# jessicabonnie/dandd

Hardware: AMD Instinct MI355X
Metric: Gbp/s sketched over k-sweep (higher is better)
Workload: dtype u64; 1 GPU; cfg2: 10 x 50 Mbp synthetic FASTA on this GPU (10 over 1 GPU(s)) resident in HBM, HLL log2m=14, k-sweep 4-40 (K=37), leaf sketches + root union + all cardinalities + delta; genomes_per_gpu=10, bases_per_genome=50000000, kmin=4, kmax=40, log2m=14, parallelism=genomes sharded over 1 GPU(s)

## Files before the change

dandd_amd/build.py:

```python
import os
import subprocess
import sys

HERE = os.path.dirname(os.path.abspath(__file__))
CSRC = os.path.join(HERE, "csrc")
LIBDIR = os.path.join(HERE, "lib")
LIB = os.path.join(LIBDIR, "libdandd_hip.so")
SOURCES = ["dd_api.hip", "dd_k2_api.hip", "dd_exact_api.hip", "dd_ingest.hip", "dd_plan.hip", "dd_pack.hip", "dd_sweep.hip", "dd_union.hip", "dd_gram.hip", "dd_leaveout.hip", "dd_extend.hip", "dd_subsets.hip", "dd_pscan.hip", "dd_synth.hip", "dd_exact.hip", "dd_exact_sched.hip", "dd_ginflate.hip", "dd_fastq.hip"]
HEADERS = ["dd_common.h", "dd_ctx.h", "dd_io.h", "dd_inflate.h", "dd_kernels.h", "dd_plan.h", os.path.join("..", "..", "include", "dandd_hip.h")]
FLAGS = [
    "-O3",
    "--offload-arch=gfx950",
    "-std=c++17",
    "-fPIC",
    "-shared",
    "-ffp-contract=off",
    "-Wall",
    "-Wno-unused-function",
]


def hipcc():
    for cand in (os.environ.get("HIPCC"), "/opt/rocm/bin/hipcc", "hipcc"):
        if cand and (os.path.isabs(cand) and os.path.exists(cand) or not os.path.isabs(cand)):
            return cand
    raise RuntimeError("hipcc not found")


OBJDIR = os.path.join(HERE, "build", "obj")
COMPILE_FLAGS = [f for f in FLAGS if f != "-shared"]


def needs_build():
    if not os.path.exists(LIB):
        return True
    t = os.path.getmtime(LIB)
    deps = [os.path.join(CSRC, s) for s in SOURCES + HEADERS] + [os.path.abspath(__file__)]
    return any(os.path.getmtime(d) > t for d in deps)


BINDIR = os.path.join(HERE, "bin")
CLI = os.path.join(BINDIR, "dashing")
CLI_SRC = os.path.join(CSRC, "dd_cli.c")
FUSED_PARALLEL = os.path.join(BINDIR, "fused", "parallel")


def build_cli(force=False):
    inc = os.path.join(HERE, "..", "include")
    deps = [CLI_SRC, os.path.join(inc, "dandd_hip.h"), LIB]
    if (not force and os.path.exists(CLI) and os.path.exists(FUSED_PARALLEL)
            and all(os.path.getmtime(d) <= min(os.path.getmtime(CLI), os.path.getmtime(FUSED_PARALLEL)) for d in deps)):
        return CLI
    os.makedirs(os.path.dirname(FUSED_PARALLEL), exist_ok=True)
    cmd = [os.environ.get("CC", "gcc"), "-std=c99", "-O2", "-Wall", "-Wextra", "-pedantic", "-I" + inc, CLI_SRC, "-o", CLI + ".tmp",
           "-L" + LIBDIR, "-ldandd_hip", "-lz", "-Wl,-rpath,$ORIGIN/../lib", "-Wl,-rpath,$ORIGIN/../../lib", "-Wl,-rpath,/opt/rocm/lib",
           "-Wl,-rpath-link," + LIBDIR]
    subprocess.check_call(cmd)
    os.replace(CLI + ".tmp", CLI)
    import shutil
    shutil.copy2(CLI, FUSED_PARALLEL + ".tmp")
    os.replace(FUSED_PARALLEL + ".tmp", FUSED_PARALLEL)
    return CLI


def _stale(obj, src):
    if not os.path.exists(obj):
        return True
    t = os.path.getmtime(obj)
    return any(os.path.getmtime(d) > t for d in [src, os.path.abspath(__file__)] + [os.path.join(CSRC, h) for h in HEADERS])


def build(force=False, extra=(), verbose=False, jobs=None):
    if not force and not needs_build():
        return LIB
    os.makedirs(LIBDIR, exist_ok=True)
    os.makedirs(OBJDIR, exist_ok=True)
    cc = hipcc()
    todo, objs = [], []
    for s in SOURCES:
        src, obj = os.path.join(CSRC, s), os.path.join(OBJDIR, s.replace(".hip", ".o"))
        objs.append(obj)
        if force or extra or _stale(obj, src):
            todo.append([cc] + COMPILE_FLAGS + list(extra) + ["-c", src, "-o", obj])
    jobs = jobs or max(1, min(len(todo), (os.cpu_count() or 2) - 1, int(os.environ.get("DD_BUILD_JOBS", "6"))))
    running = []
    for cmd in todo:
        if verbose:
            print(" ".join(cmd), file=sys.stderr)
        running.append((cmd, subprocess.Popen(cmd, cwd=CSRC)))
        while len([1 for _, p in running if p.poll() is None]) >= jobs:
            running[0][1].wait()
            running = [r for r in running if r[1].poll() is None] + [r for r in running if r[1].poll() not in (None, 0)]
            if any(p.poll() not in (None, 0) for _, p in running):
                break
    bad = [cmd for cmd, p in running if p.wait() != 0]
    if bad:
        raise subprocess.CalledProcessError(1, bad[0])
    link = [cc, "--offload-arch=gfx950", "-shared", "-fPIC", "-o", LIB + ".tmp"] + objs + ["-lz", "-ldl", "-lpthread"]
    if verbose:
        print(" ".join(link), file=sys.stderr)
    subprocess.check_call(link, cwd=CSRC)
    os.replace(LIB + ".tmp", LIB)
    return LIB


if __name__ == "__main__":
    extra = []
    if "--save-temps" in sys.argv:
        os.makedirs(OBJDIR, exist_ok=True)
        extra += ["-save-temps=obj"]
    build(force="--force" in sys.argv, extra=extra, verbose=True)
    print(LIB)
    print(build_cli(force="--force" in sys.argv))
```

dandd_amd/csrc/dd_sweep.hip:

```cpp
#include "dd_common.h"
#include "dd_kernels.h"

#include <atomic>

namespace dd {
namespace {

extern __shared__ __attribute__((aligned(16))) uint8_t g_lds[];

DD_D uint32_t ffbh(uint32_t x) {
    uint32_t r;
    asm("v_ffbh_u32 %0, %1" : "=v"(r) : "v"(x));
    return r;
}
DD_D uint32_t mul_lo(uint32_t a, uint32_t c) {
    uint32_t r;
    asm("v_mul_lo_u32 %0, %1, %2" : "=v"(r) : "v"(a), "s"(c));
    return r;
}
template <int SH>
DD_D uint64_t lshl_add64(uint64_t a, uint64_t b) {
    uint64_t r;
    asm("v_lshl_add_u64 %0, %1, %2, %3" : "=v"(r) : "v"(a), "n"(SH), "v"(b));
    return r;
}
template <bool HI_ZERO>
DD_D uint64_t mul64_c32(uint64_t x, uint32_t C, uint64_t addend) {
    const uint32_t lo = (uint32_t)x, hi = (uint32_t)(x >> 32);
    const uint64_t pr = (uint64_t)lo * C + addend;
    if (HI_ZERO) return pr;
    const uint32_t ph = (uint32_t)(pr >> 32) + mul_lo(hi, C);
    return ((uint64_t)ph << 32) | (uint32_t)pr;
}

template <bool HI_ZERO>
DD_D uint64_t wang64_fast(uint64_t x) {
    x = mul64_c32<HI_ZERO>(x, 0x1FFFFFu, ~0ull);
    x ^= x >> 24;
    x = mul64_c32<false>(x, 265u, 0ull);
    x ^= x >> 14;
    x = lshl_add64<2>(lshl_add64<2>(x, x), x);
    x ^= x >> 28;
    return lshl_add64<0>(x << 31, x);
}

DD_D void lds_starts_at_zero() {
    if ((uint32_t)(uintptr_t)(__attribute__((address_space(3))) uint8_t*)g_lds != 0u) __builtin_trap();
}

struct RegsLds {
    uint32_t slot;
    using Addr = uint32_t;
    DD_D Addr at(uint32_t hi, int p) const { return __builtin_amdgcn_alignbit(slot, hi, 32 - p); }
    DD_D static uint32_t shift(Addr a) { return (a & 3u) * 8u; }
    DD_D uint32_t bound(Addr a) const { return *(const __attribute__((address_space(3))) uint8_t*)(uintptr_t)a; }
    DD_D static uint32_t load32(Addr a) { return *(const __attribute__((address_space(3))) uint32_t*)(uintptr_t)(a & ~3u); }
    DD_D static uint32_t cas32(Addr a, uint32_t expect, uint32_t desired) {
        return atomicCAS(reinterpret_cast<uint32_t*>(g_lds + (a & ~3u)), expect, desired);
    }
};
struct RegsGlobal {
    uint8_t* base;
    using Addr = uint8_t*;
    DD_D Addr at(uint32_t hi, int p) const { return base + (hi >> (32 - p)); }
    DD_D static uint32_t shift(Addr a) { return ((uint32_t)(uintptr_t)a & 3u) * 8u; }
    DD_D static uint8_t* word(Addr a) {
        return static_cast<uint8_t*>(__builtin_assume_aligned(a - ((uintptr_t)a & 3u), 4));
    }
    DD_D uint32_t bound(Addr a) const { return gload1_fresh(a); }
    DD_D static uint32_t load32(Addr a) { return gload4_fresh(word(a)); }
    DD_D static uint32_t cas32(Addr a, uint32_t expect, uint32_t desired) { return gcas32(word(a), expect, desired); }
};

DD_D uint4 load16_fresh(const uint8_t* p) {
    const uint8_t* q = static_cast<const uint8_t*>(__builtin_assume_aligned(p, 16));
    const unsigned long long a = gload8_fresh(q), b = gload8_fresh(q + 8);
    return make_uint4((uint32_t)a, (uint32_t)(a >> 32), (uint32_t)b, (uint32_t)(b >> 32));
}
DD_D uint32_t load4_fresh(const uint32_t* p) { return gload4_fresh(p); }

struct Probe {
    uint32_t hi, lz, hiw, lo;
};
DD_D Probe probe(uint64_t h, int p) {
    const uint32_t hi = (uint32_t)(h >> 32), lo = (uint32_t)h;
    Probe r;
    r.hi = hi;
    r.hiw = __builtin_amdgcn_alignbit(hi, lo, 32 - p);
    r.lz = ffbh(r.hiw);
    r.lo = lo;
    return r;
}
DD_D uint32_t rho_of(const Probe& q, int p) {
    uint32_t rho = q.lz + 1;
    if (__builtin_expect(__any(q.hiw == 0), 0)) {
        if (q.hiw == 0) rho = 33u + (uint32_t)__builtin_clz((q.lo << p) | (1u << (p - 1)));
    }
    return rho;
}
template <typename R>
DD_D uint32_t cas_raise(typename R::Addr a, uint32_t old, uint32_t rho) {
    const uint32_t sh = R::shift(a);
    while (true) {
        const uint32_t cur = (old >> sh) & 0xFFu;
        if (rho <= cur) return cur;
        const uint32_t prev = R::cas32(a, old, old + ((rho - cur) << sh));
        if (prev == old) return rho;
        old = prev;
    }
}
template <typename R>
DD_D void raise(const R&, typename R::Addr a, const Probe& q, int p) {
    (void)cas_raise<R>(a, R::load32(a), rho_of(q, p));
}

constexpr uint32_t kQueueEntries = 128;
DD_D uint32_t min4(uint32_t w) {
    const uint32_t a = w & 0xFFu, b = (w >> 8) & 0xFFu, c = (w >> 16) & 0xFFu, d = w >> 24;
    const uint32_t ab = a < b ? a : b, cd = c < d ? c : d;
    return ab < cd ? ab : cd;
}
template <typename R>
DD_D void hll_update(const R& regs, uint64_t h, int p) {
    const Probe q = probe(h, p);
    const typename R::Addr a = regs.at(q.hi, p);
    if (q.lz >= regs.bound(a)) raise(regs, a, q, p);
}
template <typename R>
DD_D void hll_update2(const R& r0, uint64_t h0, const R& r1, uint64_t h1, int p) {
    const Probe qa = probe(h0, p), qb = probe(h1, p);
    const typename R::Addr a = r0.at(qa.hi, p), b = r1.at(qb.hi, p);
    const uint32_t c0 = r0.bound(a), c1 = r1.bound(b);
    if ((qa.lz >= c0) | (qb.lz >= c1)) {
        if (qa.lz >= c0) raise(r0, a, qa, p);
        if (qb.lz >= c1) raise(r1, b, qb, p);
    }
}

DD_D uint32_t pairrev32(uint32_t x) {
    x = __builtin_bitreverse32(x);
    return ((x >> 1) & 0x55555555u) | ((x & 0x55555555u) << 1);
}
DD_D uint64_t pack64(uint32_t hi, uint32_t lo) { return ((uint64_t)hi << 32) | lo; }

template <int KC>
struct Windows;

template <>
struct Windows<0> {
    uint32_t fw = 0, rc = 0;
    DD_D void prime(const uint4& hc) {
        fw = pairrev32(hc.w);
        rc = ~hc.w;
    }
    DD_D void push(uint32_t c) {
        fw = (fw << 2) | c;
        rc = (rc >> 2) | ((3u - c) << 30);
    }
    template <bool CANON>
    DD_D uint64_t hash(int k) const {
        const uint32_t f = (k == 16) ? fw : (fw & ((1u << (2 * k)) - 1u));
        if (!CANON) return wang64_fast<true>(f);
        const uint32_t r = rc >> (32 - 2 * k);
        return wang64_fast<true>(f < r ? f : r);
    }
};

template <>
struct Windows<1> {
    uint64_t fw = 0, rc = 0;
    DD_D void prime(const uint4& hc) {
        fw = pack64(pairrev32(hc.z), pairrev32(hc.w));
        rc = ~pack64(hc.w, hc.z);
    }
    DD_D void push(uint32_t c) {
        fw = (fw << 2) | c;
        rc = (rc >> 2) | ((uint64_t)(3u - c) << 62);
    }
    template <bool CANON>
    DD_D uint64_t hash(int k) const {
        const uint32_t mhi = (k == 32) ? ~0u : ((1u << (2 * k - 32)) - 1u);
        const uint64_t f = pack64((uint32_t)(fw >> 32) & mhi, (uint32_t)fw);
        if (!CANON) return wang64_fast<false>(f);
        const uint64_t r = rc >> (64 - 2 * k);
        return wang64_fast<false>(f < r ? f : r);
    }
};

template <>
struct Windows<5> {
    uint32_t fl = 0, fh = 0, rl = 0, rh = 0;
    DD_D void prime(const uint4& hc) {
        fh = pairrev32(hc.z);
        fl = pairrev32(hc.w);
        rh = ~hc.w;
        rl = ~hc.z;
    }
    DD_D void push(uint32_t c) {
        fh = __builtin_amdgcn_alignbit(fh, fl, 30);
        fl = (fl << 2) | c;
        rl = __builtin_amdgcn_alignbit(rh, rl, 2);
        rh = (rh >> 2) | ((3u - c) << 30);
    }
    template <bool CANON>
    DD_D uint64_t hash(int k) const {
        const uint32_t mhi = (k == 32) ? ~0u : ((1u << (2 * k - 32)) - 1u);
        const uint64_t f = pack64(fh & mhi, fl);
        if (!CANON) return wang64_fast<false>(f);
        const uint64_t r = pack64(rh, rl) >> (64 - 2 * k);
        return wang64_fast<false>(f < r ? f : r);
    }
};

template <>
struct Windows<3> {
    uint64_t fl = 0, rt = 0;
    uint32_t fh = 0, rb = 0;
    DD_D void prime(const uint4& hc) {
        fl = pack64(pairrev32(hc.z), pairrev32(hc.w));
        fh = pairrev32(hc.y);
        rt = ~pack64(hc.w, hc.z);
        rb = ~hc.y;
    }
    DD_D void push(uint32_t c) {
        fh = __builtin_amdgcn_alignbit(fh, (uint32_t)(fl >> 32), 30);
        fl = (fl << 2) | c;
        rb = __builtin_amdgcn_alignbit((uint32_t)rt, rb, 2);
        rt = (rt >> 2) | ((uint64_t)(3u - c) << 62);
    }
    template <bool CANON>
    DD_D uint64_t hash(int k) const {
        const int hb = 2 * k - 64;
        const uint32_t ah = (hb == 32) ? fh : (fh & ((1u << hb) - 1u));
        uint32_t hi = ah;
        uint64_t lo = fl;
        if (CANON) {
            const uint32_t s = 96u - 2u * (uint32_t)k;
            const uint32_t r3 = (uint32_t)(rt >> 32), r2 = (uint32_t)rt;
            const uint32_t bh = r3 >> s;
            const uint64_t bl = ((uint64_t)__builtin_amdgcn_alignbit(r3, r2, s) << 32) |
                                __builtin_amdgcn_alignbit(r2, rb, s);
            const bool f_lt = (ah < bh) | ((ah == bh) & (fl < bl));
            hi = f_lt ? ah : bh;
            lo = f_lt ? fl : bl;
        }
        const uint64_t hg = (uint64_t)hi * 0x7F4A7C15u + ((uint64_t)(hi * 0x9E3779B9u) << 32);
        return wang64_fast<false>(lo ^ hg);
    }
};

template <>
struct Windows<6> {
    uint32_t f0 = 0, f1 = 0, f2 = 0;
    uint32_t r0 = 0, r1 = 0, r2 = 0;
    DD_D void prime(const uint4& hc) {
        f0 = pairrev32(hc.w);
        f1 = pairrev32(hc.z);
        f2 = pairrev32(hc.y);
        r2 = ~hc.w;
        r1 = ~hc.z;
        r0 = ~hc.y;
    }
    DD_D void push(uint32_t c) {
        f2 = __builtin_amdgcn_alignbit(f2, f1, 30);
        f1 = __builtin_amdgcn_alignbit(f1, f0, 30);
        f0 = (f0 << 2) | c;
        r0 = __builtin_amdgcn_alignbit(r1, r0, 2);
        r1 = __builtin_amdgcn_alignbit(r2, r1, 2);
        r2 = (r2 >> 2) | ((3u - c) << 30);
    }
    template <bool CANON>
    DD_D uint64_t hash(int k) const {
        const int hb = 2 * k - 64;
        const uint32_t ah = (hb == 32) ? f2 : (f2 & ((1u << hb) - 1u));
        const uint64_t fl = pack64(f1, f0);
        uint32_t hi = ah;
        uint64_t lo = fl;
        if (CANON) {
            const uint32_t s = 96u - 2u * (uint32_t)k;
            const uint32_t bh = r2 >> s;
            const uint64_t bl = pack64(__builtin_amdgcn_alignbit(r2, r1, s), __builtin_amdgcn_alignbit(r1, r0, s));
            const bool f_lt = (ah < bh) | ((ah == bh) & (fl < bl));
            hi = f_lt ? ah : bh;
            lo = f_lt ? fl : bl;
        }
        const uint64_t hg = (uint64_t)hi * 0x7F4A7C15u + ((uint64_t)(hi * 0x9E3779B9u) << 32);
        return wang64_fast<false>(lo ^ hg);
    }
};

template <>
struct Windows<7> {
    uint32_t f0 = 0, f1 = 0, f2 = 0, f3 = 0;
    uint32_t r0 = 0, r1 = 0, r2 = 0, r3 = 0;
    DD_D void prime(const uint4& hc) {
        f0 = pairrev32(hc.w);
        f1 = pairrev32(hc.z);
        f2 = pairrev32(hc.y);
        f3 = pairrev32(hc.x);
        r3 = ~hc.w;
        r2 = ~hc.z;
        r1 = ~hc.y;
        r0 = ~hc.x;
    }
    DD_D void push(uint32_t c) {
        f3 = __builtin_amdgcn_alignbit(f3, f2, 30);
        f2 = __builtin_amdgcn_alignbit(f2, f1, 30);
        f1 = __builtin_amdgcn_alignbit(f1, f0, 30);
        f0 = (f0 << 2) | c;
        r0 = __builtin_amdgcn_alignbit(r1, r0, 2);
        r1 = __builtin_amdgcn_alignbit(r2, r1, 2);
        r2 = __builtin_amdgcn_alignbit(r3, r2, 2);
        r3 = (r3 >> 2) | ((3u - c) << 30);
    }
    template <bool CANON>
    DD_D uint64_t hash(int k) const {
        const int hb = 2 * k - 96;
        const uint32_t mh = (hb == 32) ? ~0u : ((1u << hb) - 1u);
        const uint64_t ah = pack64(f3 & mh, f2);
        const uint64_t al = pack64(f1, f0);
        if (!CANON) return wang64_fast<false>(fold128(ah, al));
        const uint32_t s = 128u - 2u * (uint32_t)k;
        const uint64_t bh = pack64(r3 >> s, __builtin_amdgcn_alignbit(r3, r2, s));
        const uint64_t bl = pack64(__builtin_amdgcn_alignbit(r2, r1, s), __builtin_amdgcn_alignbit(r1, r0, s));
        const bool f_lt = (ah < bh) | ((ah == bh) & (al < bl));
        return wang64_fast<false>(fold128(f_lt ? ah : bh, f_lt ? al : bl));
    }
};

template <int KC, bool CANON, bool CHECK, typename Win, typename MakeRegs>
DD_D void sweep_token(const Win& win, int run, int kfirst, int nk, int p, const MakeRegs& slot) {
    int j = 0;
#pragma unroll 1
    for (; j + 1 < nk; j += 2) {
        const int k = kfirst + j;
        if (!CHECK || run >= k + 1)
            hll_update2(slot(j), win.template hash<CANON>(k), slot(j + 1), win.template hash<CANON>(k + 1), p);
        else if (run >= k)
            hll_update(slot(j), win.template hash<CANON>(k), p);
    }
    if (j < nk && (!CHECK || run >= kfirst + j)) hll_update(slot(j), win.template hash<CANON>(kfirst + j), p);
}

template <int KC, bool CANON>
__global__ __launch_bounds__(1024) void sweep_kernel(const SweepGenome* __restrict__ genomes,
                                                    const SweepJob* __restrict__ jobs, int p) {
    lds_starts_at_zero();
    const SweepJob job = jobs[blockIdx.x];
    const SweepGenome g = genomes[job.genome];
    const int nk = job.nk, kfirst = job.kfirst;
    const uint32_t m = 1u << p;
    const unsigned long long ntok = gload8u(g.ntok);
    uint8_t* const slab = g.regs + ((size_t)job.krow << p);

    struct TileIn {
        uint4 hc, sc;
        uint2 hb, sb;
        bool live;
    };
    auto fetch = [&](unsigned tile, TileIn& t) {
        const unsigned long long seg = (unsigned long long)tile * blockDim.x + threadIdx.x;
        t.live = tile < job.tile_end && seg * kSegTokens < ntok;
        t.hc = make_uint4(0, 0, 0, 0);
        t.hb = make_uint2(~0u, ~0u);
        t.sc = make_uint4(0, 0, 0, 0);
        t.sb = make_uint2(~0u, ~0u);
        if (!t.live) return;
        if (seg > 0) {
            t.hc = gload16(g.codes + (seg - 1) * 4);
            t.hb = gload8(g.bad + (seg - 1) * 2);
        }
        t.sc = gload16(g.codes + seg * 4);
        t.sb = gload8(g.bad + seg * 2);
    };
    TileIn next;
    fetch(job.tile_begin, next);

    {
        uint4* z = reinterpret_cast<uint4*>(g_lds);
        const uint32_t n16 = (uint32_t)nk * (m >> 4);
        for (uint32_t i = threadIdx.x; i < n16; i += blockDim.x) z[i] = load16_fresh(slab + (size_t)i * 16);
    }
    __syncthreads();

    const int kmaxg = kfirst + nk - 1;
    auto lds_slot = [](int j) { return RegsLds{(uint32_t)j}; };

    for (unsigned tile = job.tile_begin; tile < job.tile_end; ++tile) {
        const TileIn cur = next;
        fetch(tile + 1, next);
        if (!cur.live) continue;
        const uint4 hc = cur.hc, sc = cur.sc;
        const uint2 hb = cur.hb, sb = cur.sb;
        const uint32_t cw[4] = {sc.x, sc.y, sc.z, sc.w};
        Windows<KC == 2 ? 7 : KC> win;
        win.prime(hc);
        if (__all((hb.x | hb.y | sb.x | sb.y) == 0u)) {
#pragma unroll
            for (int w = 0; w < 4; ++w) {
#pragma unroll 1
                for (int i = 0; i < 16; ++i) {
                    win.push((cw[w] >> (2 * i)) & 3u);
                    sweep_token<KC, CANON, false>(win, 0, kfirst, nk, p, lds_slot);
                }
            }
            continue;
        }
        int run = hb.y ? __builtin_clz(hb.y) : 32 + (hb.x ? __builtin_clz(hb.x) : 32);
#pragma unroll
        for (int w = 0; w < 4; ++w) {
            const uint32_t bw = ((w & 2) ? sb.y : sb.x) >> ((w & 1) * 16);
#pragma unroll 1
            for (int i = 0; i < 16; ++i) {
                const uint32_t c = (cw[w] >> (2 * i)) & 3u;
                run = ((bw >> i) & 1u) ? 0 : run + 1;
                win.push(c);
                if (__all(run >= kmaxg)) sweep_token<KC, CANON, false>(win, run, kfirst, nk, p, lds_slot);
                else sweep_token<KC, CANON, true>(win, run, kfirst, nk, p, lds_slot);
            }
        }
    }
    __syncthreads();

    const uint4* l4 = reinterpret_cast<const uint4*>(g_lds);
    uint32_t* gw = reinterpret_cast<uint32_t*>(slab);
    const uint32_t n16 = (uint32_t)nk * (m >> 4);
    for (uint32_t i = threadIdx.x; i < n16; i += blockDim.x) {
        const uint4 lv = l4[i];
        const uint4 gv = load16_fresh(slab + (size_t)i * 16);
        const uint32_t l[4] = {lv.x, lv.y, lv.z, lv.w};
        const uint32_t o[4] = {gv.x, gv.y, gv.z, gv.w};
#pragma unroll
        for (int q = 0; q < 4; ++q) {
            uint32_t old = o[q];
            uint32_t mx = bmax4(old, l[q]);
            while (mx != old) {
                uint32_t prev = gcas32(&gw[4 * i + q], old, mx);
                if (prev == old) break;
                old = prev;
                mx = bmax4(old, l[q]);
            }
        }
    }
}

__constant__ int c_bitmap_off[kBitmapMaxK + 2] = {0, bitmap_offset(1), bitmap_offset(2), bitmap_offset(3),
                                                 bitmap_offset(4), bitmap_offset(5), bitmap_offset(6),
                                                 bitmap_offset(7), bitmap_offset(8), bitmap_offset(9),
                                                 kBitmapWords};
static_assert(kBitmapMaxK == 9 && bitmap_offset(9) + bitmap_words(9) == kBitmapWords &&
              kBitmapWords + kBitmapMaxK < kBitmapStride, "bitmap layout");

template <bool CANON>
__global__ __launch_bounds__(1024) __attribute__((amdgpu_num_sgpr(72))) void bitmap_kernel(const SweepGenome* __restrict__ genomes,
                                                     const SweepJob* __restrict__ jobs) {
    const SweepJob job = jobs[blockIdx.x];
    const SweepGenome g = genomes[job.genome];
    const int kfirst = job.kfirst, klast = job.kfirst + job.nk - 1;
    const unsigned long long ntok = gload8u(g.ntok);
    const int w0 = c_bitmap_off[kfirst], w1 = c_bitmap_off[klast + 1];
    uint32_t* const bits = reinterpret_cast<uint32_t*>(g_lds) - w0;
    uint32_t kmask = __builtin_amdgcn_readfirstlane(((2u << klast) - 1u) & ~((1u << kfirst) - 1u));
    uint32_t* const complete = g.bitmap + kBitmapWords;
    __shared__ uint32_t have[kBitmapMaxK + 2];
    __shared__ uint32_t flagged;
    if (threadIdx.x == 0) {
        uint32_t f = 0;
        for (int k = kfirst; k <= klast; ++k)
            if (load4_fresh(complete + k)) f |= 1u << k;
        flagged = f;
    }
    if (threadIdx.x <= kBitmapMaxK) have[threadIdx.x] = 0;
    __syncthreads();
    kmask = __builtin_amdgcn_readfirstlane(kmask & ~flagged);
    if (kmask == 0u) return;
    for (int i = w0 + (int)threadIdx.x; i < w1; i += blockDim.x) {
        const uint32_t v = load4_fresh(&g.bitmap[i]);
        bits[i] = v;
        if (v) {
            int k = kfirst;
            for (int j = kfirst + 1; j <= klast; ++j) k = (i >= c_bitmap_off[j]) ? j : k;
            atomicAdd(&have[k], (uint32_t)__builtin_popcount(v));
        }
    }
    __syncthreads();
    auto all_of = [](int k) { return CANON ? (1u << (2 * k - 1)) + ((k & 1) ? 0u : (1u << (k - 1))) : (1u << (2 * k)); };
    for (int k = kfirst; k <= klast; ++k) {
        if (have[k] == all_of(k)) {
            kmask &= ~(1u << k);
            if (threadIdx.x == 0) gstore4(complete + k, 1u);
        }
    }
    kmask = __builtin_amdgcn_readfirstlane(kmask);
    if (kmask == 0u) return;

    const int prime = klast - 1;
    for (unsigned tile = job.tile_begin; tile < job.tile_end; ++tile) {
        const unsigned long long seg = (unsigned long long)tile * blockDim.x + threadIdx.x;
        if (seg * kSegTokens >= ntok) continue;
        uint32_t fw = 0, rc = 0;
        int run = 0;
        if (seg > 0) {
            const uint4 hc = gload16(g.codes + (seg - 1) * 4);
            const uint2 hb = gload8(g.bad + (seg - 1) * 2);
            const uint32_t cw = hc.w, bw = hb.y >> 16;
#pragma unroll 1
            for (int i = 16 - prime; i < 16; ++i) {
                const uint32_t c = (cw >> (2 * i)) & 3u;
                run = ((bw >> i) & 1u) ? 0 : run + 1;
                fw = (fw << 2) | c;
                rc = (rc >> 2) | ((3u - c) << 30);
            }
        }
        const uint4 sc = gload16(g.codes + seg * 4);
        const uint2 sb = gload8(g.bad + seg * 2);
        const uint32_t cws[4] = {sc.x, sc.y, sc.z, sc.w};
#pragma unroll
        for (int w = 0; w < 4; ++w) {
            const uint32_t bw = ((w & 2) ? sb.y : sb.x) >> ((w & 1) * 16);
#pragma unroll 1
            for (int i = 0; i < 16; ++i) {
                const uint32_t c = (cws[w] >> (2 * i)) & 3u;
                run = ((bw >> i) & 1u) ? 0 : run + 1;
                fw = (fw << 2) | c;
                rc = (rc >> 2) | ((3u - c) << 30);
                uint32_t xs[kBitmapMaxK + 1], seen[kBitmapMaxK + 1];
                uint32_t all_seen = 1u;
#pragma unroll
                for (int k = 1; k <= kBitmapMaxK; ++k) {
                    if (!((kmask >> k) & 1u)) continue;
                    uint32_t x = fw & ((1u << (2 * k)) - 1u);
                    if (CANON) {
                        const uint32_t r = rc >> (32 - 2 * k);
                        x = x < r ? x : r;
                    }
                    xs[k] = x;
                    seen[k] = bits[bitmap_offset(k) + (x >> 5)];
                    all_seen &= seen[k] >> (x & 31u);
                }
                if (!(all_seen & 1u)) {
#pragma unroll
                    for (int k = 1; k <= kBitmapMaxK; ++k) {
                        if (!((kmask >> k) & 1u) || run < k) continue;
                        if (!((seen[k] >> (xs[k] & 31u)) & 1u))
                            atomicOr(&bits[bitmap_offset(k) + (xs[k] >> 5)], 1u << (xs[k] & 31u));
                    }
                }
            }
        }
    }
    __syncthreads();
    if (threadIdx.x <= kBitmapMaxK) have[threadIdx.x] = 0;
    __syncthreads();
    for (int i = w0 + (int)threadIdx.x; i < w1; i += blockDim.x) {
        const uint32_t mine = bits[i], theirs = load4_fresh(&g.bitmap[i]);
        if (mine & ~theirs) gor32(&g.bitmap[i], mine);
        int k = kfirst;
        for (int j = kfirst + 1; j <= klast; ++j) k = (i >= c_bitmap_off[j]) ? j : k;
        if (mine | theirs) atomicAdd(&have[k], (uint32_t)__builtin_popcount(mine | theirs));
    }
    __syncthreads();
    if (threadIdx.x >= (unsigned)kfirst && threadIdx.x <= (unsigned)klast && have[threadIdx.x] == all_of((int)threadIdx.x))
        gstore4(complete + threadIdx.x, 1u);
}

template <bool CANON_UNUSED>
__global__ __launch_bounds__(1024) void bitmap_finish_kernel(const SweepGenome* __restrict__ genomes,
                                                            int kfirst, int kmin, int p, int tile_log2) {
    lds_starts_at_zero();
    const SweepGenome g = genomes[blockIdx.y];
    const int k = kfirst + (int)blockIdx.x;
    const uint32_t tile = 1u << tile_log2, b = blockIdx.z;
    const uint32_t* bm = g.bitmap + c_bitmap_off[k];
    const int nw = c_bitmap_off[k + 1] - c_bitmap_off[k];
    if (gridDim.z > 1 && nw <= 512) {
        if (b != 0) return;
        uint8_t* const row = g.regs + ((size_t)(k - kmin) << p);
        for (int w = threadIdx.x; w < nw; w += blockDim.x) {
            uint32_t v = gload4(bm + w);
            while (v) {
                const uint32_t bit = (uint32_t)__builtin_ctz(v);
                v &= v - 1;
                hll_update(RegsGlobal{row}, wang64_fast<true>(((uint32_t)w << 5) | bit), p);
            }
        }
        return;
    }
    uint8_t* const out = g.regs + ((size_t)(k - kmin) << p) + (size_t)b * tile;
    uint4* z = reinterpret_cast<uint4*>(g_lds);
    for (uint32_t i = threadIdx.x; i < (tile >> 4); i += blockDim.x) z[i] = make_uint4(0, 0, 0, 0);
    __syncthreads();
    for (int w = threadIdx.x; w < nw; w += blockDim.x) {
        uint32_t v = gload4(bm + w);
        while (v) {
            const uint32_t bit = (uint32_t)__builtin_ctz(v);
            v &= v - 1;
            const Probe q = probe(wang64_fast<true>(((uint32_t)w << 5) | bit), p);
            const uint32_t idx = q.hi >> (32 - p);
            if ((idx >> tile_log2) != b) continue;
            const uint32_t a = idx & (tile - 1u), rho = rho_of(q, p);
            const uint32_t wd = RegsLds::load32(a);
            if (rho > ((wd >> RegsLds::shift(a)) & 0xFFu)) (void)cas_raise<RegsLds>(a, wd, rho);
        }
    }
    __syncthreads();
    const uint4* l4 = reinterpret_cast<const uint4*>(g_lds);
    for (uint32_t i = threadIdx.x; i < (tile >> 4); i += blockDim.x) gstore16(out + (size_t)i * 16, l4[i]);
}


template <bool CANON>
DD_D uint32_t bigmap_index(uint32_t fw, uint32_t rc, int k) {
    if (!CANON) return fw;
    if (k & 1) {
        const uint32_t y = ((fw >> k) & 1u) ? rc : fw;
        return ((y >> (k + 1)) << k) | (y & ((1u << k) - 1u));
    }
    return fw < rc ? fw : rc;
}
template <bool CANON>
DD_D uint32_t bigmap_kmer(uint32_t idx, int k) {
    if (!CANON || !(k & 1)) return idx;
    const uint32_t y = ((idx >> k) << (k + 1)) | (idx & ((1u << k) - 1u));
    uint32_t r = __brev(y);
    r = ((r >> 1) & 0x55555555u) | ((r & 0x55555555u) << 1);
    r = (~r) >> (32 - 2 * k);
    return y < r ? y : r;
}

template <bool CANON>
__global__ __launch_bounds__(1024) void bigmap_kernel(const SweepGenome* __restrict__ genomes, const SweepJob* __restrict__ jobs) {
    const SweepJob job = jobs[blockIdx.x];
    const SweepGenome g = genomes[job.genome];
    const int k = job.kfirst;
    const uint32_t slice = (uint32_t)job.slice;
    const unsigned long long ntok = gload8u(g.ntok);
    uint32_t* const home = g.bigmap + bigmap_offset_words(k, CANON) + (size_t)slice * kBigmapSliceWords;
    uint32_t* const bits = reinterpret_cast<uint32_t*>(g_lds);
    for (int i = threadIdx.x; i < kBigmapSliceWords; i += blockDim.x) bits[i] = load4_fresh(home + i);
    __syncthreads();
    const uint32_t mask = (1u << (2 * k)) - 1u;
    const int top = 2 * k - 2, prime = k - 1;
    for (unsigned tile = job.tile_begin; tile < job.tile_end; ++tile) {
        const unsigned long long seg = (unsigned long long)tile * blockDim.x + threadIdx.x;
        if (seg * kSegTokens >= ntok) continue;
        uint32_t fw = 0, rc = 0;
        int run = 0;
        if (seg > 0) {
            const uint4 hc = gload16(g.codes + (seg - 1) * 4);
            const uint2 hb = gload8(g.bad + (seg - 1) * 2);
            const uint32_t cw = hc.w, bw = hb.y >> 16;
#pragma unroll 1
            for (int i = 16 - prime; i < 16; ++i) {
                const uint32_t c = (cw >> (2 * i)) & 3u;
                run = ((bw >> i) & 1u) ? 0 : run + 1;
                fw = ((fw << 2) | c) & mask;
                rc = (rc >> 2) | ((3u - c) << top);
            }
        }
        const uint4 sc = gload16(g.codes + seg * 4);
        const uint2 sb = gload8(g.bad + seg * 2);
        const uint32_t cws[4] = {sc.x, sc.y, sc.z, sc.w};
        auto record = [&](uint32_t idx, bool ok) {
            if ((idx >> 20) == slice && ok) {
                const uint32_t at = (idx & 0xFFFFFu) >> 5, bit = 1u << (idx & 31u);
                if (!(bits[at] & bit)) atomicOr(&bits[at], bit);
            }
        };
        if (__all((sb.x | sb.y) == 0u && run >= prime)) {
#pragma unroll
            for (int w = 0; w < 4; ++w) {
#pragma unroll 4
                for (int i = 0; i < 16; ++i) {
                    const uint32_t c = (cws[w] >> (2 * i)) & 3u;
                    fw = ((fw << 2) | c) & mask;
                    rc = (rc >> 2) | ((3u - c) << top);
                    record(bigmap_index<CANON>(fw, rc, k), true);
                }
            }
            continue;
        }
#pragma unroll
        for (int w = 0; w < 4; ++w) {
            const uint32_t bw = ((w & 2) ? sb.y : sb.x) >> ((w & 1) * 16);
#pragma unroll 4
            for (int i = 0; i < 16; ++i) {
                const uint32_t c = (cws[w] >> (2 * i)) & 3u;
                run = ((bw >> i) & 1u) ? 0 : run + 1;
                fw = ((fw << 2) | c) & mask;
                rc = (rc >> 2) | ((3u - c) << top);
                record(bigmap_index<CANON>(fw, rc, k), run >= k);
            }
        }
    }
    __syncthreads();
    for (int i = threadIdx.x; i < kBigmapSliceWords; i += blockDim.x) {
        const uint32_t mine = bits[i];
        if (mine && (mine & ~load4_fresh(home + i))) gor32(home + i, mine);
    }
}

template <bool CANON>
__global__ __launch_bounds__(1024) void bigmap_finish_kernel(const SweepGenome* __restrict__ genomes,
                                                            int kfirst, int kmin, int p, int tile_log2) {
    lds_starts_at_zero();
    const SweepGenome g = genomes[blockIdx.y];
    const int k = kfirst + (int)blockIdx.x;
    const uint32_t tile = 1u << tile_log2, b = blockIdx.z;
    uint8_t* const out = g.regs + ((size_t)(k - kmin) << p) + (size_t)b * tile;
    uint4* z = reinterpret_cast<uint4*>(g_lds);
    for (uint32_t i = threadIdx.x; i < (tile >> 4); i += blockDim.x) z[i] = make_uint4(0, 0, 0, 0);
    __syncthreads();
    const uint32_t* bm = g.bigmap + bigmap_offset_words(k, CANON);
    const uint32_t nw = (uint32_t)bigmap_slices(k, CANON) * kBigmapSliceWords;
    for (uint32_t w = threadIdx.x; w < nw; w += blockDim.x) {
        uint32_t v = gload4(bm + w);
        while (v) {
            const uint32_t bit = (uint32_t)__builtin_ctz(v);
            v &= v - 1;
// ... 701 lines not shown
```

Measured before the change: 36.17 Gbp/s.

## Derive k-mer windows from precomputed token slices instead of incremental shifting

```diff
diff --git a/dandd_amd/build.py b/dandd_amd/build.py
--- a/dandd_amd/build.py
+++ b/dandd_amd/build.py
@@ -7,7 +7,7 @@
 LIBDIR = os.path.join(HERE, "lib")
 LIB = os.path.join(LIBDIR, "libdandd_hip.so")
 SOURCES = ["dd_api.hip", "dd_k2_api.hip", "dd_exact_api.hip", "dd_ingest.hip", "dd_plan.hip", "dd_pack.hip", "dd_sweep.hip", "dd_union.hip", "dd_gram.hip", "dd_leaveout.hip", "dd_extend.hip", "dd_subsets.hip", "dd_pscan.hip", "dd_synth.hip", "dd_exact.hip", "dd_exact_sched.hip", "dd_ginflate.hip", "dd_fastq.hip"]
-HEADERS = ["dd_common.h", "dd_ctx.h", "dd_io.h", "dd_inflate.h", "dd_kernels.h", "dd_plan.h", os.path.join("..", "..", "include", "dandd_hip.h")]
+HEADERS = ["dd_common.h", "dd_ctx.h", "dd_io.h", "dd_inflate.h", "dd_kernels.h", "dd_plan.h", "dd_slices.h", os.path.join("..", "..", "include", "dandd_hip.h")]
 FLAGS = [
     "-O3",
     "--offload-arch=gfx950",
diff --git a/dandd_amd/csrc/dd_slices.h b/dandd_amd/csrc/dd_slices.h
--- /dev/null
+++ b/dandd_amd/csrc/dd_slices.h
@@ -0,0 +1,41 @@
+#pragma once
+#include <stdint.h>
+
+#ifndef DD_HD
+#define DD_HD inline
+#endif
+
+namespace dd {
+
+DD_HD uint32_t funnel32(uint32_t hi, uint32_t lo, uint32_t s) {
+#if defined(__HIP_DEVICE_COMPILE__)
+    return __builtin_amdgcn_alignbit(hi, lo, s);
+#else
+    return (uint32_t)((((uint64_t)hi << 32) | lo) >> (s & 31u));
+#endif
+}
+
+DD_HD uint32_t pairrev32(uint32_t x) {
+#if defined(__HIP_DEVICE_COMPILE__)
+    x = __builtin_bitreverse32(x);
+    return ((x >> 1) & 0x55555555u) | ((x & 0x55555555u) << 1);
+#else
+    x = ((x >> 2) & 0x33333333u) | ((x & 0x33333333u) << 2);
+    x = ((x >> 4) & 0x0F0F0F0Fu) | ((x & 0x0F0F0F0Fu) << 4);
+    x = ((x >> 8) & 0x00FF00FFu) | ((x & 0x00FF00FFu) << 8);
+    return (x >> 16) | (x << 16);
+#endif
+}
+
+struct TokenSlices {
+    uint32_t R[8], N[8];
+    DD_HD void prepare(const uint32_t (&C)[8]) {
+        for (int m = 0; m < 8; ++m) R[m] = pairrev32(C[7 - m]);
+        for (int j = 0; j < 7; ++j) N[j] = ~funnel32(C[j + 1], C[j], 2);
+        N[7] = ~(C[7] >> 2);
+    }
+    DD_HD uint32_t fw(int w, int q, int i) const { return funnel32(R[4 - w + q], R[3 - w + q], 30u - 2u * (uint32_t)i); }
+    DD_HD uint32_t rc(int w, int q, int i) const { return funnel32(N[w + 1 + q], N[w + q], 2u * (uint32_t)i); }
+};
+
+}
diff --git a/dandd_amd/csrc/dd_sweep.hip b/dandd_amd/csrc/dd_sweep.hip
--- a/dandd_amd/csrc/dd_sweep.hip
+++ b/dandd_amd/csrc/dd_sweep.hip
@@ -1,5 +1,6 @@
 #include "dd_common.h"
 #include "dd_kernels.h"
+#include "dd_slices.h"
 
 #include <atomic>
 
@@ -50,13 +51,21 @@
 
 struct RegsLds {
     uint32_t slot;
+    uint32_t down;
     using Addr = uint32_t;
-    DD_D Addr at(uint32_t hi, int p) const { return __builtin_amdgcn_alignbit(slot, hi, 32 - p); }
+    DD_D static uint32_t index_shift(int p) {
+        uint32_t v;
+        asm("v_mov_b32 %0, %1" : "=v"(v) : "s"(32 - p));
+        return v;
+    }
+    DD_D Addr at(uint32_t hi, int) const { return __builtin_amdgcn_alignbit(slot, hi, down); }
     DD_D static uint32_t shift(Addr a) { return (a & 3u) * 8u; }
     DD_D uint32_t bound(Addr a) const { return *(const __attribute__((address_space(3))) uint8_t*)(uintptr_t)a; }
     DD_D static uint32_t load32(Addr a) { return *(const __attribute__((address_space(3))) uint32_t*)(uintptr_t)(a & ~3u); }
     DD_D static uint32_t cas32(Addr a, uint32_t expect, uint32_t desired) {
-        return atomicCAS(reinterpret_cast<uint32_t*>(g_lds + (a & ~3u)), expect, desired);
+        __hip_atomic_compare_exchange_strong((__attribute__((address_space(3))) uint32_t*)(uintptr_t)(a & ~3u), &expect, desired,
+                                             __ATOMIC_RELAXED, __ATOMIC_RELAXED, __HIP_MEMORY_SCOPE_WORKGROUP);
+        return expect;
     }
 };
 struct RegsGlobal {
@@ -137,10 +146,6 @@
     }
 }
 
-DD_D uint32_t pairrev32(uint32_t x) {
-    x = __builtin_bitreverse32(x);
-    return ((x >> 1) & 0x55555555u) | ((x & 0x55555555u) << 1);
-}
 DD_D uint64_t pack64(uint32_t hi, uint32_t lo) { return ((uint64_t)hi << 32) | lo; }
 
 template <int KC>
@@ -157,6 +162,10 @@
         fw = (fw << 2) | c;
         rc = (rc >> 2) | ((3u - c) << 30);
     }
+    DD_D void take(const TokenSlices& s, int w, int i) {
+        fw = s.fw(w, 0, i);
+        rc = s.rc(w, 3, i);
+    }
     template <bool CANON>
     DD_D uint64_t hash(int k) const {
         const uint32_t f = (k == 16) ? fw : (fw & ((1u << (2 * k)) - 1u));
@@ -169,13 +178,9 @@
 template <>
 struct Windows<1> {
     uint64_t fw = 0, rc = 0;
-    DD_D void prime(const uint4& hc) {
-        fw = pack64(pairrev32(hc.z), pairrev32(hc.w));
-        rc = ~pack64(hc.w, hc.z);
-    }
-    DD_D void push(uint32_t c) {
-        fw = (fw << 2) | c;
-        rc = (rc >> 2) | ((uint64_t)(3u - c) << 62);
+    DD_D void take(const TokenSlices& s, int w, int i) {
+        fw = pack64(s.fw(w, 1, i), s.fw(w, 0, i));
+        rc = pack64(s.rc(w, 3, i), s.rc(w, 2, i));
     }
     template <bool CANON>
     DD_D uint64_t hash(int k) const {
@@ -216,17 +221,11 @@
 struct Windows<3> {
     uint64_t fl = 0, rt = 0;
     uint32_t fh = 0, rb = 0;
-    DD_D void prime(const uint4& hc) {
-        fl = pack64(pairrev32(hc.z), pairrev32(hc.w));
-        fh = pairrev32(hc.y);
-        rt = ~pack64(hc.w, hc.z);
-        rb = ~hc.y;
-    }
-    DD_D void push(uint32_t c) {
-        fh = __builtin_amdgcn_alignbit(fh, (uint32_t)(fl >> 32), 30);
-        fl = (fl << 2) | c;
-        rb = __builtin_amdgcn_alignbit((uint32_t)rt, rb, 2);
-        rt = (rt >> 2) | ((uint64_t)(3u - c) << 62);
+    DD_D void take(const TokenSlices& s, int w, int i) {
+        fl = pack64(s.fw(w, 1, i), s.fw(w, 0, i));
+        fh = s.fw(w, 2, i);
+        rt = pack64(s.rc(w, 3, i), s.rc(w, 2, i));
+        rb = s.rc(w, 1, i);
     }
     template <bool CANON>
     DD_D uint64_t hash(int k) const {
@@ -313,6 +312,10 @@
         r2 = __builtin_amdgcn_alignbit(r3, r2, 2);
         r3 = (r3 >> 2) | ((3u - c) << 30);
     }
+    DD_D void take(const TokenSlices& s, int w, int i) {
+        f0 = s.fw(w, 0, i), f1 = s.fw(w, 1, i), f2 = s.fw(w, 2, i), f3 = s.fw(w, 3, i);
+        r0 = s.rc(w, 0, i), r1 = s.rc(w, 1, i), r2 = s.rc(w, 2, i), r3 = s.rc(w, 3, i);
+    }
     template <bool CANON>
     DD_D uint64_t hash(int k) const {
         const int hb = 2 * k - 96;
@@ -330,16 +333,17 @@
 
 template <int KC, bool CANON, bool CHECK, typename Win, typename MakeRegs>
 DD_D void sweep_token(const Win& win, int run, int kfirst, int nk, int p, const MakeRegs& slot) {
-    int j = 0;
+    int npairs = nk >> 1, tail = nk & 1;
+    asm volatile("" : "+s"(npairs), "+s"(tail));
 #pragma unroll 1
-    for (; j + 1 < nk; j += 2) {
-        const int k = kfirst + j;
+    for (int jp = 0; jp < npairs; ++jp) {
+        const int j = 2 * jp, k = kfirst + j;
         if (!CHECK || run >= k + 1)
             hll_update2(slot(j), win.template hash<CANON>(k), slot(j + 1), win.template hash<CANON>(k + 1), p);
         else if (run >= k)
             hll_update(slot(j), win.template hash<CANON>(k), p);
     }
-    if (j < nk && (!CHECK || run >= kfirst + j)) hll_update(slot(j), win.template hash<CANON>(kfirst + j), p);
+    if (tail && (!CHECK || run >= kfirst + nk - 1)) hll_update(slot(nk - 1), win.template hash<CANON>(kfirst + nk - 1), p);
 }
 
 template <int KC, bool CANON>
@@ -350,7 +354,9 @@
     const SweepGenome g = genomes[job.genome];
     const int nk = job.nk, kfirst = job.kfirst;
     const uint32_t m = 1u << p;
-    const unsigned long long ntok = gload8u(g.ntok);
+    const unsigned long long ntok_v = gload8u(g.ntok);
+    const unsigned long long ntok = pack64(__builtin_amdgcn_readfirstlane((uint32_t)(ntok_v >> 32)),
+                                           __builtin_amdgcn_readfirstlane((uint32_t)ntok_v));
     uint8_t* const slab = g.regs + ((size_t)job.krow << p);
 
     struct TileIn {
@@ -384,7 +390,8 @@
     __syncthreads();
 
     const int kmaxg = kfirst + nk - 1;
-    auto lds_slot = [](int j) { return RegsLds{(uint32_t)j}; };
+    const uint32_t down = RegsLds::index_shift(p);
+    auto lds_slot = [down](int j) { return RegsLds{(uint32_t)j, down}; };
 
     for (unsigned tile = job.tile_begin; tile < job.tile_end; ++tile) {
         const TileIn cur = next;
@@ -392,15 +399,16 @@
         if (!cur.live) continue;
         const uint4 hc = cur.hc, sc = cur.sc;
         const uint2 hb = cur.hb, sb = cur.sb;
-        const uint32_t cw[4] = {sc.x, sc.y, sc.z, sc.w};
+        const uint32_t cw[8] = {hc.x, hc.y, hc.z, hc.w, sc.x, sc.y, sc.z, sc.w};
+        TokenSlices sl;
+        sl.prepare(cw);
         Windows<KC == 2 ? 7 : KC> win;
-        win.prime(hc);
         if (__all((hb.x | hb.y | sb.x | sb.y) == 0u)) {
 #pragma unroll
             for (int w = 0; w < 4; ++w) {
 #pragma unroll 1
                 for (int i = 0; i < 16; ++i) {
-                    win.push((cw[w] >> (2 * i)) & 3u);
+                    win.take(sl, w, i);
                     sweep_token<KC, CANON, false>(win, 0, kfirst, nk, p, lds_slot);
                 }
             }
@@ -412,9 +420,8 @@
             const uint32_t bw = ((w & 2) ? sb.y : sb.x) >> ((w & 1) * 16);
 #pragma unroll 1
             for (int i = 0; i < 16; ++i) {
-                const uint32_t c = (cw[w] >> (2 * i)) & 3u;
                 run = ((bw >> i) & 1u) ? 0 : run + 1;
-                win.push(c);
+                win.take(sl, w, i);
                 if (__all(run >= kmaxg)) sweep_token<KC, CANON, false>(win, run, kfirst, nk, p, lds_slot);
                 else sweep_token<KC, CANON, true>(win, run, kfirst, nk, p, lds_slot);
             }
```

Result: no change. 36.12 Gbp/s (-0.1%).
